# CVMI-Lab/DODA

Measured on AMD Instinct MI355X. Metric: active-voxels/sec fwd+bwd SparseConv U-Net, ScanNet 2cm, higher is better.
Workload: dtype bf16; 1 GPU; cfgs/scannet SparseConv U-Net training step (voxel pooling + fwd + CE + bwd + SGD), 2 cm voxels, 4 scenes/GPU x ~150000 active voxels, random-init weights; global_batch=4, voxels_per_gpu=601279, points_per_gpu=781042, parallelism=dp1, n_classes=20, grad_sync=deferred multi-layer wgrad + bucketed all-reduce, collectives=none (single process), prefetch_gate=off, grad_exchange=no process group

## Files before the change

doda_amd/csrc/spconv_gather.hip:

```cpp
#include <cstdio>
#include "common.hpp"
#include "tilebook.hpp"
#include "spconv_common.hpp"
#include "wgrad_backends.hpp"
#include <stdlib.h>

namespace {

struct F32 {
    typedef float elem;
    typedef f32x4 frag;
    static __device__ __forceinline__ frag zero() { return (frag){0.f, 0.f, 0.f, 0.f}; }
    static __device__ __forceinline__ elem from_float(float f) { return f; }
    static __device__ __forceinline__ float to_float(elem e) { return e; }
    static __device__ __forceinline__ void mma(f32x4 &acc, const frag &w, const frag &x) {
        mma_f32_k16<false>(acc, __builtin_bit_cast(u32x4, w), __builtin_bit_cast(u32x4, x));
    }
    static __device__ __forceinline__ void store4(elem *p, const f32x4 &v) {
        *reinterpret_cast<f32x4 *>(p) = v;
    }
};

struct BF16 {
    typedef unsigned short elem;
    typedef s16x4 frag;
    static __device__ __forceinline__ frag zero() { return (frag){0, 0, 0, 0}; }
    static __device__ __forceinline__ elem from_float(float f) { return f2bf(f); }
    static __device__ __forceinline__ float to_float(elem e) { return __uint_as_float((unsigned)e << 16); }
    static __device__ __forceinline__ void mma(f32x4 &acc, const frag &w, const frag &x) {
        acc = __builtin_amdgcn_mfma_f32_16x16x16bf16_1k(w, x, acc, 0, 0, 0);
    }
    static __device__ __forceinline__ void store4(elem *p, const f32x4 &v) {
        s16x4 o;
#pragma unroll
        for (int q = 0; q < 4; ++q) o[q] = (short)f2bf(v[q]);
        *reinterpret_cast<s16x4 *>(p) = o;
    }
};

template <class T>
__global__ __launch_bounds__(256) void pack_weights(const float *__restrict__ w, int K, int kc,
                                                    int nc, int n_chunk, int NB, int wl,
                                                    typename T::frag *__restrict__ packed) {
    const long long total = (long long)K * n_chunk * NB * 64;
    const long long e = (long long)blockIdx.x * blockDim.x + threadIdx.x;
    if (e >= total) return;
    const int lane = (int)(e & 63);
    long long r = e >> 6;
    const int nb = (int)(r % NB); r /= NB;
    const int cc = (int)(r % n_chunk);
    const int o = (int)(r / n_chunk);
    const int i = lane & 15, g = lane >> 4;
    const int col = nb * 16 + i;
    typename T::frag v;
#pragma unroll
    for (int q = 0; q < 4; ++q) {
        const int c = cc * 16 + 4 * g + q;
        float f = 0.f;
        if (c < kc && col < nc) {
            if (wl == 0) f = w[((long long)o * kc + c) * nc + col];
            else f = w[((long long)(wl == 2 ? K - 1 - o : o) * nc + col) * kc + c];
        }
        v[q] = T::from_float(f);
    }
    packed[e] = v;
}

__device__ __forceinline__ u32x4_t pack_wide_frag(const float *__restrict__ w, int K, int kc, int nc,
                                                  int wl, int o, int cc, int nb, int lane) {
    const int i = lane & 15, g = lane >> 4;
    const int col = nb * 16 + i;
    unsigned short h[8];
#pragma unroll
    for (int q = 0; q < 8; ++q) {
        const int c = cc * 32 + 8 * g + q;
        float f = 0.f;
        if (c < kc && col < nc) {
            if (wl == 0) f = w[((unsigned)o * (unsigned)kc + (unsigned)c) * (unsigned)nc + (unsigned)col];
            else f = w[((unsigned)(wl == 2 ? K - 1 - o : o) * (unsigned)nc + (unsigned)col) * (unsigned)kc + (unsigned)c];
        }
        h[q] = f2bf(f);
    }
    u32x4_t r;
#pragma unroll
    for (int q = 0; q < 4; ++q) r[q] = (unsigned)h[2 * q] | ((unsigned)h[2 * q + 1] << 16);
    return r;
}

__global__ __launch_bounds__(256) void pack_weights_wide(const float *__restrict__ w, int K, int kc,
                                                         int nc, int n_chunk, int NB, int wl,
                                                         u32x4_t *__restrict__ packed, int pair) {
    const long long e = (long long)blockIdx.x * blockDim.x + threadIdx.x;
    if (pair) {
        if (e >= (long long)K * NB * 32) return;
        const long long r = e >> 5;
        packed[e] = pack_wide_frag(w, K, kc, nc, wl, (int)(r / NB), 0, (int)(r % NB), (int)(e & 31));
        return;
    }
    const long long total = (long long)K * n_chunk * NB * 64;
    if (e >= total) return;
    const int lane = (int)(e & 63);
    long long r = e >> 6;
    const int nb = (int)(r % NB); r /= NB;
    const int cc = (int)(r % n_chunk);
    const int o = (int)(r / n_chunk);
    packed[e] = pack_wide_frag(w, K, kc, nc, wl, o, cc, nb, lane);
}

struct PackDesc {
    const float *w;
    void *out;
    int K, kc, nc, layout, elem_bytes, n_chunk, NB, pad;
};

template <class T>
__device__ __forceinline__ void pack_one(const PackDesc &d, long long e) {
    const int lane = (int)(e & 63);
    const unsigned r = (unsigned)(e >> 6), r1 = r / (unsigned)d.NB;
    const int nb = (int)(r - r1 * (unsigned)d.NB);
    const int o = (int)(r1 / (unsigned)d.n_chunk), cc = (int)(r1 - (unsigned)o * (unsigned)d.n_chunk);
    const int i = lane & 15, g = lane >> 4;
    const int col = nb * 16 + i;
    typename T::frag v;
#pragma unroll
    for (int q = 0; q < 4; ++q) {
        const int c = cc * 16 + 4 * g + q;
        float f = 0.f;
        if (c < d.kc && col < d.nc) {
            if ((d.layout & 3) == 0) f = d.w[((long long)o * d.kc + c) * d.nc + col];
            else f = d.w[((long long)((d.layout & 3) == 2 ? d.K - 1 - o : o) * d.nc + col) * d.kc + c];
        }
        v[q] = T::from_float(f);
    }
    reinterpret_cast<typename T::frag *>(d.out)[e] = v;
}

__global__ __launch_bounds__(256) void pack_weights_multi(const PackDesc *__restrict__ descs,
                                                          const int *__restrict__ blk_end, int n_desc) {
    int lo = 0, hi = n_desc - 1;
    while (lo < hi) {
        const int mid = (lo + hi) >> 1;
        if ((int)blockIdx.x < blk_end[mid]) hi = mid; else lo = mid + 1;
    }
    const PackDesc d = descs[lo];
    const int first = lo == 0 ? 0 : blk_end[lo - 1];
    const unsigned e = (unsigned)(blockIdx.x - first) * 256u + threadIdx.x;
    if (d.layout & 0x20) {
        if (e >= (unsigned)d.K * (unsigned)d.NB * 32u) return;
        const unsigned r = e >> 5, o = r / (unsigned)d.NB;
        reinterpret_cast<u32x4_t *>(d.out)[e] =
            pack_wide_frag(d.w, d.K, d.kc, d.nc, d.layout & 3, (int)o, 0, (int)(r - o * (unsigned)d.NB), (int)(e & 31));
        return;
    }
    const unsigned total = (unsigned)d.K * (unsigned)d.n_chunk * (unsigned)d.NB * 64u;
    if (e >= total) return;
    if (d.layout & 0x10) {
        const unsigned r = e >> 6, r1 = r / (unsigned)d.NB, nb = r - r1 * (unsigned)d.NB;
        const unsigned o = r1 / (unsigned)d.n_chunk, cc = r1 - o * (unsigned)d.n_chunk;
        reinterpret_cast<u32x4_t *>(d.out)[e] =
            pack_wide_frag(d.w, d.K, d.kc, d.nc, d.layout & 3, (int)o, (int)cc, (int)nb, (int)(e & 63));
    } else if (d.elem_bytes == 4) pack_one<F32>(d, e);
    else pack_one<BF16>(d, e);
}

constexpr int MAX_K = 27;

template <class T, int NBW, int S>
__global__ __launch_bounds__(256) void conv_gather(const typename T::elem *__restrict__ x, int kc,
                                                   const typename T::frag *__restrict__ wp, int nc,
                                                   int NB, const int32_t *__restrict__ tbl, int ld,
                                                   int K, int n_out,
                                                   typename T::elem *__restrict__ y, int vec_ok,
                                                   const typename T::elem *__restrict__ res) {
    typedef typename T::frag frag;
    typedef typename T::elem elem;
    constexpr int TM = 4 * 16 * S;
    __shared__ int32_t idx_tile[MAX_K * TM];

    const int lane = threadIdx.x & 63, wid = threadIdx.x >> 6;
    const int i = lane & 15, g = lane >> 4;
    const int n_nbg = (NB + NBW - 1) / NBW;
    const int item = xcd_work_item(blockIdx.x, gridDim.x);
    const long long r0 = (long long)(item / n_nbg) * TM;
    const int nb0 = (item % n_nbg) * NBW;

    for (int e = threadIdx.x; e < K * TM; e += 256) {
        const int o = e / TM, r = e - o * TM;
        idx_tile[e] = (r0 + r < n_out) ? tbl[(long long)o * ld + r0 + r] : -1;
    }
    doda_sync();

    const int wrow = wid * 16 * S;
    if (r0 + wrow >= n_out) return;

    unsigned int active = 0;
    for (int o = 0; o < K; ++o) {
        bool any = false;
#pragma unroll
        for (int s = 0; s < S; ++s) any |= idx_tile[o * TM + wrow + s * 16 + i] >= 0;
        if (__ballot(any) != 0ull) active |= 1u << o;
    }
    active = __builtin_amdgcn_readfirstlane(active);

    f32x4 acc[S][NBW];
#pragma unroll
    for (int s = 0; s < S; ++s)
#pragma unroll
        for (int nb = 0; nb < NBW; ++nb) acc[s][nb] = (f32x4){0.f, 0.f, 0.f, 0.f};

    const int n_chunk = (kc + 15) / 16;

    auto load_unit = [&](int o, int cc, frag (&xa)[S], frag (&wb)[NBW]) {
        const int c0 = cc * 16 + 4 * g;
#pragma unroll
        for (int s = 0; s < S; ++s) {
            const int idx = idx_tile[o * TM + wrow + s * 16 + i];
            xa[s] = T::zero();
            if (idx >= 0 && c0 < kc) {
                const elem *row = x + (long long)idx * kc + c0;
                if (vec_ok) {
                    xa[s] = *reinterpret_cast<const frag *>(row);
                } else {
#pragma unroll
                    for (int q = 0; q < 4; ++q)
                        if (c0 + q < kc) xa[s][q] = row[q];
                }
            }
        }
        const frag *wrow_p = wp + (((long long)o * n_chunk + cc) * NB + nb0) * 64 + lane;
#pragma unroll
        for (int nb = 0; nb < NBW; ++nb)
            if (nb0 + nb < NB) wb[nb] = wrow_p[nb * 64];
    };
    auto mma_unit = [&](const frag (&xa)[S], const frag (&wb)[NBW]) {
#pragma unroll
        for (int nb = 0; nb < NBW; ++nb)
#pragma unroll
            for (int s = 0; s < S; ++s) T::mma(acc[s][nb], wb[nb], xa[s]);
    };
    auto advance = [&](int &o, int &cc) -> bool {
        if (++cc < n_chunk) return true;
        cc = 0;
        if (active == 0) return false;
        o = __builtin_ctz(active);
        active &= active - 1;
        return true;
    };

    if (active != 0) {
        frag xa0[S], xa1[S], wb0[NBW], wb1[NBW];
#pragma unroll
        for (int nb = 0; nb < NBW; ++nb) { wb0[nb] = T::zero(); wb1[nb] = T::zero(); }
        int o = __builtin_ctz(active), cc = 0;
        active &= active - 1;
        load_unit(o, cc, xa0, wb0);
        for (;;) {
            const bool m1 = advance(o, cc);
            if (m1) load_unit(o, cc, xa1, wb1);
            mma_unit(xa0, wb0);
            if (!m1) break;
            const bool m0 = advance(o, cc);
            if (m0) load_unit(o, cc, xa0, wb0);
            mma_unit(xa1, wb1);
            if (!m0) break;
        }
    }

#pragma unroll
    for (int s = 0; s < S; ++s) {
        const long long t = r0 + wrow + s * 16 + i;
        if (t < n_out) {
#pragma unroll
            for (int nb = 0; nb < NBW; ++nb) {
                const int col = (nb0 + nb) * 16 + 4 * g;
                if (nb0 + nb < NB) {
                    elem *p = y + t * nc + col;
// ... 761 lines not shown
```

doda_amd/csrc/spconv_wgrad.hip:

```cpp
#include "wgrad_common.hpp"
#include <string.h>
#include <mutex>
#include <vector>

namespace {

constexpr int RT = 64;
constexpr int MAX_OGW = 7;
constexpr int PAD = 8;

struct F32 {
    typedef float elem;
    typedef f32x4 frag;
    typedef f32x4 vec;
    static constexpr int VEC = 4;
    static constexpr int KSTEPS = RT / 4;
    typedef float kfrag;
    template <int STRIDE>
    static __device__ __forceinline__ void frags(const elem *tile, int g, int i, int col0, kfrag (&out)[KSTEPS]) {
#pragma unroll
        for (int ks = 0; ks < KSTEPS; ++ks) out[ks] = tile[(ks * 4 + g) * STRIDE + col0 + i];
    }
    static __device__ __forceinline__ f32x4 mma(kfrag a, kfrag b, f32x4 c) {
        return __builtin_amdgcn_mfma_f32_16x16x4f32(a, b, c, 0, 0, 0);
// ... 94 lines not shown

    const long long r_begin = (long long)chunk * rows_per_chunk;
    long long r_end = r_begin + rows_per_chunk;
    if (r_end > n_rows) r_end = n_rows;

    elem *my_a = a_tile[wid];

    typedef typename T::vec vec;
    constexpr int VEC = T::VEC, NVA = TA * 16 / VEC, NVB = TB * 16 / VEC;
    auto load_vec = [&](const elem *p, const elem *safe, int c, int cmax, bool ok) -> vec {
        const bool live = ok && c < cmax;
        if constexpr (VOK) {
            return *reinterpret_cast<const vec *>(live ? p : safe);
        } else {
            vec v = vec{};
            if (live) {
                elem tmp[VEC];
#pragma unroll
                for (int q = 0; q < VEC; ++q) tmp[q] = (c + q < cmax) ? p[q] : (elem)0;
                v = *reinterpret_cast<const vec *>(tmp);
            }
            return v;
        }
    };
    auto gather_row = [&](int idx, vec (&dst)[NVA]) {
#pragma unroll
        for (int f = 0; f < NVA; ++f) {
            const int c = ca0 + f * VEC;
            dst[f] = load_vec(a + (long long)(idx >= 0 ? idx : 0) * ca + c, a, c, ca, idx >= 0);
        }
    };

    constexpr int NDY = (RT * NVB + 255) / 256;
    vec dy_reg[NDY];
    int idx_n[OGW];
    auto load_dy = [&](long long r0) {
#pragma unroll
        for (int k = 0; k < NDY; ++k) {
            const int e = threadIdx.x + k * 256;
            const int r = e / NVB, f = e - r * NVB;
            const long long row = r0 + r;
            const int c = cb0 + f * VEC;
            dy_reg[k] = load_vec(b + (row < r_end ? row : 0) * cb + c, b, c, cb, e < RT * NVB && row < r_end);
        }
    };
    auto load_idx = [&](long long r0) {
#pragma unroll
        for (int oo = 0; oo < OGW; ++oo) {
            const int o = o_base + wid + 4 * oo;
            const long long row = r0 + lane;
            idx_n[oo] = tbl[(o < K && row < r_end) ? (long long)o * ld + row : 0];
        }
    };

    vec rows_cur[NVA], rows_nxt[NVA];
    if (r_begin < r_end) {
        load_dy(r_begin);
        load_idx(r_begin);
        gather_row((o_base + wid < K && r_begin + lane < r_end) ? idx_n[0] : -1, rows_cur);
    }
    for (long long r0 = r_begin; r0 < r_end; r0 += RT) {
        doda_sync();
#pragma unroll
        for (int k = 0; k < NDY; ++k) {
            const int e = threadIdx.x + k * 256;
            if (e < RT * NVB) {
                const int r = e / NVB, f = e - r * NVB;
                const bool live = r0 + r < r_end && cb0 + f * VEC < cb;
                *reinterpret_cast<vec *>(&b_tile[r * SB + f * VEC]) = (VOK && !live) ? vec{} : dy_reg[k];
            }
        }
        int idx[OGW];
#pragma unroll
        for (int oo = 0; oo < OGW; ++oo)
            idx[oo] = (o_base + wid + 4 * oo < K && r0 + lane < r_end) ? idx_n[oo] : -1;
        const bool more = r0 + RT < r_end;
        if (more) {
            load_dy(r0 + RT);
            load_idx(r0 + RT);
        }
        doda_sync();
        kfrag bf[TB][T::KSTEPS];
#pragma unroll
        for (int y_ = 0; y_ < TB; ++y_) T::template frags<SB>(b_tile, g, i, y_ * 16, bf[y_]);

#pragma unroll
        for (int oo = 0; oo < OGW; ++oo) {
            if (oo + 1 < OGW) gather_row(idx[oo + 1], rows_nxt);
            else if (more) gather_row((o_base + wid < K && r0 + RT + lane < r_end) ? idx_n[0] : -1, rows_nxt);
            if (__ballot(idx[oo] >= 0) != 0ull) {
#pragma unroll
                for (int f = 0; f < NVA; ++f) {
                    const bool live = idx[oo] >= 0 && ca0 + f * VEC < ca;
                    *reinterpret_cast<vec *>(&my_a[lane * SA + f * VEC]) = (VOK && !live) ? vec{} : rows_cur[f];
                }
                __builtin_amdgcn_wave_barrier();
#pragma unroll
                for (int x_ = 0; x_ < TA; ++x_) {
                    kfrag af[T::KSTEPS];
                    T::template frags<SA>(my_a, g, i, x_ * 16, af);
#pragma unroll
                    for (int ks = 0; ks < T::KSTEPS; ++ks)
#pragma unroll
                        for (int y_ = 0; y_ < TB; ++y_)
                            acc[oo][x_][y_] = T::mma(af[ks], bf[y_][ks], acc[oo][x_][y_]);
                }
                __builtin_amdgcn_wave_barrier();
            }
#pragma unroll
            for (int f = 0; f < NVA; ++f) rows_cur[f] = rows_nxt[f];
        }
    }

    float *out = partial + (long long)chunk * K * ca * cb;
#pragma unroll
    for (int oo = 0; oo < OGW; ++oo) {
        const int o = o_base + wid + 4 * oo;
        if (o < K) {
#pragma unroll
            for (int x_ = 0; x_ < TA; ++x_)
#pragma unroll
                for (int y_ = 0; y_ < TB; ++y_)
#pragma unroll
                    for (int r = 0; r < 4; ++r) {
                        const int ci = ca0 + x_ * 16 + 4 * g + r, co = cb0 + y_ * 16 + i;
                        if (ci < ca && co < cb)
                            out[((long long)o * ca + ci) * cb + co] = acc[oo][x_][y_][r];
                    }
        }
    }
}

struct WJob {
    const void *a, *b;
    const int32_t *tbl;
    float *out;
    int ca, cb, ld, K, n_rows, rows_per_chunk, n_tag, n_tbg, n_og, blk_end;
};
using doda_wgrad::RJob;

template <class T, int TA, int TB, int OGW, bool VOK>
__global__ __launch_bounds__(256) void wgrad_multi_kernel(const WJob *__restrict__ jobs, int n_jobs) {
    const int j = find_job<WJob, &WJob::blk_end>(jobs, n_jobs, (int)blockIdx.x);
    const WJob d = jobs[j];
    const int first = j == 0 ? 0 : jobs[j - 1].blk_end;
    wgrad_body<T, TA, TB, OGW, VOK>((const typename T::elem *)d.a, d.ca, (const typename T::elem *)d.b, d.cb,
                                    d.tbl, d.ld, d.K, d.n_rows, d.rows_per_chunk, d.n_tag, d.n_tbg, d.n_og,
                                    d.out, (int)blockIdx.x - first);
}

__global__ __launch_bounds__(256) void wgrad_reduce_multi(const RJob *__restrict__ jobs, int n_jobs) {
    const int j = find_job<RJob, &RJob::blk_end>(jobs, n_jobs, (int)blockIdx.x);
    const RJob d = jobs[j];
    wgrad_fold((int)blockIdx.x - (j == 0 ? 0 : jobs[j - 1].blk_end), d.R, d.n_quad, d.n_quad, d.dw, d.accumulate,
               [&](long long q) { return d.partial + q; });
}

__global__ __launch_bounds__(256) void wgrad_reduce(const float *__restrict__ partial, int R,
                                                    long long n_elem, float *__restrict__ dw,
                                                    int accumulate = 0) {
    __shared__ float part[16][17];
    const int el = threadIdx.x & 15, rl = threadIdx.x >> 4;
    const long long e = (long long)blockIdx.x * 16 + el;
    float s = 0.f;
    if (e < n_elem)
        for (int r = rl; r < R; r += 16) s += partial[(long long)r * n_elem + e];
    part[rl][el] = s;
    doda_sync();
    if (rl == 0 && e < n_elem) {
        float t = 0.f;
#pragma unroll
        for (int r = 0; r < 16; ++r) t += part[r][el];
        dw[e] = accumulate ? dw[e] + t : t;
    }
}


static_assert(WP_RT == RT && WP_MAX_OGW == MAX_OGW, "wgrad_plan.hpp restates these constants");

template <class T, WgradPolicy P, class... Tile>
void launch_multi_variant(WgradTiles<Tile...>, const DensePlan &p, int total_blocks, const WJob *jobs_dev, int n, hipStream_t s) {
    const auto go = [&](auto tile) {
        typedef decltype(tile) Tl;
        if constexpr (dense_compiled(P, Tl::TA, Tl::TB, Tl::OGW))
            if (p.TA == Tl::TA && p.TB == Tl::TB && p.OGW == Tl::OGW)
                with_bool(p.vok, [&](auto vok) {
                    hipLaunchKernelGGL((wgrad_multi_kernel<T, Tl::TA, Tl::TB, Tl::OGW, decltype(vok)::value>), dim3(total_blocks), dim3(256), 0, s, jobs_dev, n);
                });
    };
    (go(Tile{}), ...);
}

struct Staging {
    std::mutex mu;
    void *host = nullptr;
    size_t cap = 0;
    hipEvent_t ev = nullptr;
    int ev_dev = -1;
    bool pending = false;
};
Staging g_staging;

namespace doda_dense {

struct Plan {
    std::vector<int> idx;
    std::vector<DensePlan> jp;
    std::vector<size_t> ws_off;
    std::vector<char> red;
    struct Group { int first, count, blocks, rep; };
    std::vector<Group> groups;
    std::vector<int> order, blk_end;
    int status = DODA_OK;
    size_t partial_bytes = 0, desc_bytes = 0;
    int n_reduce = 0;
};

Plan plan(const doda_wgrad_job *jobs, const std::vector<int> &idx) {
    Plan p;
    p.idx = idx;
    p.jp.resize(idx.size());
    p.ws_off.resize(idx.size());
    p.red.resize(idx.size());
    std::vector<int> keys;
    for (size_t k = 0; k < idx.size(); ++k) {
        DensePlan &jp = p.jp[k];
        const doda_wgrad_job &j = jobs[idx[k]];
        jp.key = -1;
        if (!dense_valid(j)) { p.status = DODA_ERR_INVALID; continue; }
        jp = plan_dense(j, doda_wgrad::switches());
        if (!dense_compiled(jp.policy, jp.TA, jp.TB, jp.OGW) && p.status == DODA_OK) p.status = DODA_ERR_UNSUPPORTED;
        const bool quads = (long long)j.K * j.ca * j.cb % 4 == 0 && (uintptr_t)j.dw % 16 == 0;
        p.red[k] = !dense_needs_partial(jp, j) ? 0 : quads ? 1 : 2;
        p.ws_off[k] = p.partial_bytes;
        p.partial_bytes += dense_partial_bytes(jp, j);
        p.n_reduce += p.red[k] == 1;
        bool seen = false;
        for (int key : keys) seen |= key == jp.key;
        if (!seen) keys.push_back(jp.key);
    }
    for (int key : keys) {
        Plan::Group g{(int)p.order.size(), 0, 0, -1};
        for (size_t k = 0; k < idx.size(); ++k) {
            if (p.jp[k].key != key) continue;
            if (g.rep < 0) g.rep = (int)k;
            g.blocks += p.jp[k].blocks;
            p.order.push_back((int)k);
            p.blk_end.push_back(g.blocks);
            ++g.count;
        }
        p.groups.push_back(g);
    }
    p.desc_bytes = p.order.size() * sizeof(WJob);
    return p;
}

void write_desc(const Plan &p, const doda_wgrad_job *jobs, char *part, void *desc, std::vector<RJob> &reduce, int *reduce_blocks) {
    WJob *wj = (WJob *)desc;
    for (size_t q = 0; q < p.order.size(); ++q) {
        const int k = p.order[q];
        const DensePlan &jp = p.jp[k];
        const doda_wgrad_job &j = jobs[p.idx[k]];
        WJob d;
        d.a = j.a; d.b = j.b; d.tbl = j.tbl;
        d.out = p.red[k] ? (float *)(part + p.ws_off[k]) : j.dw;
        d.ca = j.ca; d.cb = j.cb; d.ld = j.ld; d.K = j.K; d.n_rows = j.n_rows;
        d.rows_per_chunk = jp.rows_per_chunk; d.n_tag = jp.n_tag; d.n_tbg = jp.n_tbg; d.n_og = jp.n_og;
        d.blk_end = p.blk_end[q];
        wj[q] = d;
    }
    for (size_t k = 0; k < p.idx.size(); ++k)
        if (p.red[k] == 1) doda_wgrad::push_reduce(reduce, reduce_blocks, part + p.ws_off[k], jobs[p.idx[k]], p.jp[k].R);
}

int launch(const Plan &p, const void *desc_dev, hipStream_t s) {
    const WJob *wj_dev = (const WJob *)desc_dev;
    for (const Plan::Group &g : p.groups) {
        const DensePlan &q = p.jp[g.rep];
        char name[64];
        dense_name(q, name, sizeof name);
        doda_wgrad::trace(name, g.blocks, 256, g.count);
        if (q.policy == WP_F32S) launch_multi_variant<F32S, WP_F32S>(DenseTiles{}, q, g.blocks, wj_dev + g.first, g.count, s);
        else if (q.policy == WP_F32) launch_multi_variant<F32, WP_F32>(DenseTiles{}, q, g.blocks, wj_dev + g.first, g.count, s);
        else launch_multi_variant<BF16, WP_BF16>(DenseTiles{}, q, g.blocks, wj_dev + g.first, g.count, s);
    }
    return doda_check_launch();
}

int launch_scalar_reduce(const Plan &p, const doda_wgrad_job *jobs, char *part, hipStream_t s) {
    for (size_t k = 0; k < p.idx.size(); ++k) {
        const doda_wgrad_job &j = jobs[p.idx[k]];
        const long long n_elem = (long long)j.K * j.ca * j.cb;
        if (p.red[k] != 2) continue;
        doda_wgrad::trace("wgrad_reduce", div_up(n_elem, 16), 256, 1);
        hipLaunchKernelGGL(wgrad_reduce, dim3(div_up(n_elem, 16)), dim3(256), 0, s, (const float *)(part + p.ws_off[k]), p.jp[k].R,
                           n_elem, j.dw, (j.flags & DODA_WGRAD_ACCUMULATE) ? 1 : 0);
    }
    return doda_check_launch();
}

}

struct CallPlan {
    std::vector<int> cls;
    doda_dense::Plan dense;
    doda_pairs::Plan pairs;
    doda_wdma::Plan tile;
// ... 101 lines not shown
```

doda_amd/csrc/spconv_wwide.hip:

```cpp
#include "wgrad_common.hpp"
#include "tilebook.hpp"
#include <string.h>
#include <algorithm>
#include <vector>

namespace {

constexpr int WW_WAVES = 16;
constexpr int WW_MO = (TB_K + WW_WAVES - 1) / WW_WAVES;
constexpr int WW_LIST_BYTES = TB_UMAX * 4;
constexpr int ww_stage_bytes(int ta, int tb) { return TB_T * 32 * tb + (TB_LMAX + 1) * 32 * ta; }
constexpr int WW_STAGE_MAX = ww_stage_bytes(3, 3);
constexpr int WW_SMEM = WW_LIST_BYTES + TB_LIDX_BYTES + WW_STAGE_MAX;
static_assert(WW_SMEM <= 160 * 1024, "one workgroup per CU");
static_assert(TB_T + 1 <= TB_LMAX + 1, "the dense fallback stages 256 rows into the row slots");

struct WwJob {
    const unsigned short *x, *dy;
    const int32_t *tbl;
    const void *tb;
    float *dw, *part;
    int ca, cb, ld, n_rows, nt, ta, tb_, n_sb, P, rpc, accumulate;
    int wg_end, red_end;
    int pad;
};

__device__ __forceinline__ s16x4 ww_tr(unsigned addr) {
    return __builtin_amdgcn_ds_read_tr16_b64_v4i16((__attribute__((address_space(3))) s16x4 *)(uintptr_t)addr);
}
__device__ __forceinline__ bf16x8 ww_frag(unsigned a_lo, unsigned a_hi) {
    const s16x4 lo = ww_tr(a_lo), hi = ww_tr(a_hi);
    return __builtin_bit_cast(bf16x8, __builtin_shufflevector(lo, hi, 0, 1, 2, 3, 4, 5, 6, 7));
}

template <int TA, int TB>
__device__ void ww_body(const WwJob &d, int local, unsigned char *smem) {
    constexpr int RA = 32 * TA, RB = 32 * TB;
    constexpr int CIS = 16 * TA, COS = 16 * TB, SLICE = TB_K * CIS * COS;
    const int tid = threadIdx.x, wid = __builtin_amdgcn_readfirstlane(tid >> 6);
    const int lane = tid & 63, i = lane & 15, g = lane >> 4, q4 = i >> 2, c4 = i & 3;
    const int slice = local / d.P, p = local - slice * d.P;
    const int sa = slice / d.n_sb, sb = slice - sa * d.n_sb;
    const int ca0 = sa * CIS, cb0 = sb * COS;
    const int r_begin = p * d.rpc, r_end = min(d.n_rows, r_begin + d.rpc);
    const int tile_begin = r_begin / TB_T, tile_end = (r_end - 1) / TB_T + 1;
    static_assert(ww_stage_bytes(TA, TB) <= WW_STAGE_MAX, "staging buffers");
    const int32_t *tb_ulist = (const int32_t *)d.tb;
    const uint32_t *tb_lidx = (const uint32_t *)(tb_ulist + (size_t)d.nt * TB_UMAX);
    const int32_t *tb_ucount = (const int32_t *)(tb_lidx + (size_t)d.nt * (TB_LIDX_BYTES / 4));

    int32_t *list_s = reinterpret_cast<int32_t *>(smem);
    const unsigned *lidx_s = reinterpret_cast<const unsigned *>(smem + WW_LIST_BYTES);
    unsigned char *dy_s = smem + WW_LIST_BYTES + TB_LIDX_BYTES;
    unsigned char *rows_s = dy_s + TB_T * RB;
    const unsigned dy_base = (unsigned)(uintptr_t)dy_s, rows_base = (unsigned)(uintptr_t)rows_s;

    f32x4 acc[WW_MO][TA][TB];
#pragma unroll
    for (int m = 0; m < WW_MO; ++m)
#pragma unroll
        for (int a = 0; a < TA; ++a)
#pragma unroll
            for (int b = 0; b < TB; ++b) acc[m][a][b] = (f32x4){0.f, 0.f, 0.f, 0.f};

    auto multiply = [&](bool dense, int only_o, int ks_begin, int ks_end) {
#pragma unroll 1
        for (int ks = ks_begin; ks < ks_end; ++ks) {
            const int r = 32 * ks + 8 * g + q4;
            bf16x8 bf[TB];
#pragma unroll
            for (int b = 0; b < TB; ++b) {
                const unsigned a0 = dy_base + (unsigned)(r * RB + b * 32 + c4 * 8);
                bf[b] = ww_frag(a0, a0 + 4u * RB);
            }
#pragma unroll
            for (int m = 0; m < WW_MO; ++m) {
                const int o = wid + WW_WAVES * m;
                if (o >= TB_K || (dense && o != only_o)) continue;
                unsigned s0, s1;
                if (dense) {
                    s0 = (unsigned)(r + 1);
                    s1 = (unsigned)(r + 5);
                } else {
                    const unsigned *pl = lidx_s + tb_lplane(o) * TB_T;
                    const unsigned sh = tb_lshift(o);
                    s0 = __builtin_amdgcn_ubfe(pl[tb_lpos(r)], sh, 10u);
                    s1 = __builtin_amdgcn_ubfe(pl[tb_lpos(r + 4)], sh, 10u);
                }
                const unsigned x0 = rows_base + s0 * RA + (unsigned)(c4 * 8), x1 = rows_base + s1 * RA + (unsigned)(c4 * 8);
#pragma unroll
                for (int a = 0; a < TA; ++a) {
                    const bf16x8 af = ww_frag(x0 + 32u * a, x1 + 32u * a);
#pragma unroll
                    for (int b = 0; b < TB; ++b)
                        acc[m][a][b] = __builtin_amdgcn_mfma_f32_16x16x32_bf16(af, bf[b], acc[m][a][b], 0, 0, 0);
                }
            }
        }
    };

    for (int e = tid; e < RA / 16; e += 1024) reinterpret_cast<u32x4 *>(rows_s)[e] = (u32x4){0u, 0u, 0u, 0u};
    for (int tile = tile_begin; tile < tile_end; ++tile) {
        const int t0 = tile * TB_T;
        const int ks_begin = max(0, (r_begin - t0) / 32), ks_end = min(TB_T / 32, (r_end - t0 + 31) / 32);
        const int ucount = tb_ucount[tile];
        const bool listed = ucount <= TB_LMAX;
        if (listed) {
            const int e = (tid & 3) * 256 + ((tid >> 7) & 7) * 32 + ((tid >> 2) & 31);
            list_s[e] = tb_ulist[(size_t)tile * TB_UMAX + tid];
            for (int v = tid; v < TB_LIDX_BYTES / 16; v += 1024)
                reinterpret_cast<u32x4 *>(smem + WW_LIST_BYTES)[v] =
                    reinterpret_cast<const u32x4 *>(tb_lidx + (size_t)tile * (TB_LIDX_BYTES / 4))[v];
        }
        for (int v = tid; v < TB_T * (RB / 16); v += 1024) {
            const int t = v / (RB / 16), f = v - t * (RB / 16);
            u32x4 val = (u32x4){0u, 0u, 0u, 0u};
            if (t0 + t < d.n_rows) val = *reinterpret_cast<const u32x4 *>(d.dy + (size_t)(t0 + t) * d.cb + cb0 + f * 8);
            *reinterpret_cast<u32x4 *>(dy_s + t * RB + f * 16) = val;
        }
        doda_sync();
        if (listed) {
            for (int v = tid; v < ucount * (RA / 16); v += 1024) {
                const int e = v / (RA / 16), f = v - e * (RA / 16);
                const int row = list_s[e];
                *reinterpret_cast<u32x4 *>(rows_s + (e + 1) * RA + f * 16) =
                    *reinterpret_cast<const u32x4 *>(d.x + (size_t)row * d.ca + ca0 + f * 8);
            }
            doda_sync();
            multiply(false, 0, ks_begin, ks_end);
            doda_sync();
        } else {
            for (int o = 0; o < TB_K; ++o) {
                for (int v = tid; v < TB_T * (RA / 16); v += 1024) {
                    const int t = v / (RA / 16), f = v - t * (RA / 16);
                    const int row = t0 + t < d.n_rows ? d.tbl[(size_t)o * d.ld + t0 + t] : -1;
                    u32x4 val = (u32x4){0u, 0u, 0u, 0u};
                    if (row >= 0) val = *reinterpret_cast<const u32x4 *>(d.x + (size_t)row * d.ca + ca0 + f * 8);
                    *reinterpret_cast<u32x4 *>(rows_s + (t + 1) * RA + f * 16) = val;
                }
                doda_sync();
                multiply(true, o, ks_begin, ks_end);
                doda_sync();
            }
        }
    }

    float *dst = d.part + (size_t)local * SLICE;
#pragma unroll
    for (int m = 0; m < WW_MO; ++m) {
        const int o = wid + WW_WAVES * m;
        if (o >= TB_K) continue;
#pragma unroll
        for (int a = 0; a < TA; ++a)
#pragma unroll
            for (int b = 0; b < TB; ++b)
#pragma unroll
                for (int r = 0; r < 4; ++r)
                    dst[((size_t)o * CIS + a * 16 + 4 * g + r) * COS + b * 16 + i] = acc[m][a][b][r];
    }
}

__global__ __launch_bounds__(1024) void wgrad_wide(const WwJob *__restrict__ jobs, int n_jobs) {
    __shared__ __attribute__((aligned(16))) unsigned char smem[WW_SMEM];
    const int j = find_job<WwJob, &WwJob::wg_end>(jobs, n_jobs, (int)blockIdx.x);
    const WwJob d = jobs[j];
    const int local = (int)blockIdx.x - (j == 0 ? 0 : jobs[j - 1].wg_end);
#define WW_CASE(A, B) if (d.ta == A && d.tb_ == B) { ww_body<A, B>(d, local, smem); return; }
    WW_SHAPES(WW_CASE)
#undef WW_CASE
}

__global__ __launch_bounds__(256) void wgrad_wide_reduce(const WwJob *__restrict__ jobs, int n_jobs) {
    const int j = find_job<WwJob, &WwJob::red_end>(jobs, n_jobs, (int)blockIdx.x);
    const WwJob d = jobs[j];
    const int CIS = 16 * d.ta, COS = 16 * d.tb_, SLICE = TB_K * CIS * COS;
    wgrad_fold((int)blockIdx.x - (j == 0 ? 0 : jobs[j - 1].red_end), d.P, (long long)TB_K * d.ca * d.cb / 4, SLICE / 4,
               reinterpret_cast<float4 *>(d.dw), d.accumulate, [&](long long q) {
        const long long e = 4 * q;
        const int co = (int)(e % d.cb), ci = (int)((e / d.cb) % d.ca), o = (int)(e / ((long long)d.ca * d.cb));
        const int slice = (ci / CIS) * d.n_sb + co / COS;
        return reinterpret_cast<const float4 *>(d.part + ((size_t)slice * d.P) * SLICE + ((size_t)o * CIS + ci % CIS) * COS + co % COS);
    });
}

}

namespace doda_wwide {

Plan plan(const doda_wgrad_job *jobs, const std::vector<int> &idx) {
    Plan pl;
    pl.n = (int)idx.size();
    std::vector<int> order;
    for (int k = 0; k < pl.n; ++k) order.push_back(k);
    std::stable_sort(order.begin(), order.end(), [&](int a, int b) { return jobs[idx[a]].n_rows > jobs[idx[b]].n_rows; });
    std::vector<WwJob> desc;
    for (int kk : order) {
        const doda_wgrad_job &j = jobs[idx[kk]];
        WwJob d;
        d.x = (const unsigned short *)j.a; d.dy = (const unsigned short *)j.b; d.tbl = j.tbl; d.tb = j.tilebook;
        d.dw = j.dw;
        d.ca = j.ca; d.cb = j.cb; d.ld = j.ld; d.n_rows = j.n_rows; d.nt = (j.n_rows + TB_T - 1) / TB_T;
        const WideGeo g = wwide_geo(j, doda_wgrad::switches());
        d.ta = g.ta; d.tb_ = g.tb; d.rpc = g.rpc; d.P = g.P;
        d.n_sb = j.cb / (16 * d.tb_);
        d.accumulate = (j.flags & DODA_WGRAD_ACCUMULATE) ? 1 : 0;
        d.part = (float *)(uintptr_t)pl.partial_bytes;
        pl.partial_bytes += g.partial_bytes;
        pl.wgs += g.blocks;
        d.wg_end = pl.wgs;
        pl.red_blocks += doda_wgrad::reduce_blocks((long long)TB_K * j.ca * j.cb / 4, d.P);
        d.red_end = pl.red_blocks;
        d.pad = 0;
        desc.push_back(d);
    }
    pl.desc_bytes = desc.size() * sizeof(WwJob);
    pl.desc.resize(pl.desc_bytes);
    if (pl.desc_bytes) memcpy(pl.desc.data(), desc.data(), pl.desc_bytes);
    return pl;
}

size_t desc_bytes_per_job() { return sizeof(WwJob); }

void write_desc(const Plan &p, char *part, void *desc) {
    if (p.desc_bytes) memcpy(desc, p.desc.data(), p.desc_bytes);
    WwJob *d = (WwJob *)desc;
    for (int k = 0; k < p.n; ++k) d[k].part = (float *)(part + (uintptr_t)d[k].part);
}

int launch(const Plan &p, const void *desc_dev, hipStream_t s) {
    doda_wgrad::trace("wgrad_wide", p.wgs, 1024, p.n);
    hipLaunchKernelGGL(wgrad_wide, dim3(p.wgs), dim3(1024), 0, s, (const WwJob *)desc_dev, p.n);
    doda_wgrad::trace("wgrad_wide_reduce", p.red_blocks, 256, p.n);
    hipLaunchKernelGGL(wgrad_wide_reduce, dim3(p.red_blocks), dim3(256), 0, s, (const WwJob *)desc_dev, p.n);
    return doda_check_launch();
}

}
```

doda_amd/csrc/voxelize.hip:

```cpp
#include "common.hpp"

namespace {

__global__ __launch_bounds__(256) void voxel_pool_fwd(const float *__restrict__ feats,
                                                      float *__restrict__ out,
                                                      const int32_t *__restrict__ rules,
                                                      int n_rows, int row_w, int n_plane,
                                                      int average) {
    const long long total = (long long)n_rows * n_plane;
    for (long long e = (long long)blockIdx.x * blockDim.x + threadIdx.x; e < total;
         e += (long long)gridDim.x * blockDim.x) {
        const int row = (int)(e / n_plane), plane = (int)(e - (long long)row * n_plane);
        const int32_t *r = rules + (long long)row * row_w;
        const int cnt = r[0];
        const float mult = (average && cnt > 0) ? __fdiv_rn(1.0f, (float)cnt) : 1.0f;
        float acc = out[e];
        for (int i = 1; i <= cnt; ++i) {
            const float v = feats[(long long)r[i] * n_plane + plane];
            acc = __fadd_rn(acc, __fmul_rn(mult, v));
        }
        out[e] = acc;
    }
}

__global__ __launch_bounds__(256) void voxel_pool_bwd(const float *__restrict__ d_out,
                                                      float *__restrict__ d_feats,
                                                      const int32_t *__restrict__ rules,
                                                      int n_rows, int row_w, int n_plane,
                                                      int average) {
    const long long total = (long long)n_rows * n_plane;
    for (long long e = (long long)blockIdx.x * blockDim.x + threadIdx.x; e < total;
         e += (long long)gridDim.x * blockDim.x) {
        const int row = (int)(e / n_plane), plane = (int)(e - (long long)row * n_plane);
        const int32_t *r = rules + (long long)row * row_w;
        const int cnt = r[0];
        const float mult = (average && cnt > 0) ? __fdiv_rn(1.0f, (float)cnt) : 1.0f;
        const float g = __fmul_rn(mult, d_out[e]);
        for (int i = 1; i <= cnt; ++i) atomicAdd(&d_feats[(long long)r[i] * n_plane + plane], g);
    }
}

template <typename OUT>
__global__ __launch_bounds__(256) void voxel_pool_rows(const float *__restrict__ fa, int ca, const float *__restrict__ fb, int cb,
                                                       const int32_t *__restrict__ rules, int n_rows, int row_w, int average,
                                                       OUT *__restrict__ out, int c_out) {
    const long long total = (long long)n_rows * c_out;
    for (long long e = (long long)blockIdx.x * blockDim.x + threadIdx.x; e < total; e += (long long)gridDim.x * blockDim.x) {
        const int row = (int)(e / c_out), plane = (int)(e - (long long)row * c_out);
        float acc = 0.0f;
        if (plane < ca + cb) {
            const int32_t *r = rules + (long long)row * row_w;
            const int cnt = r[0];
            const float mult = (average && cnt > 0) ? __fdiv_rn(1.0f, (float)cnt) : 1.0f;
            const bool first = plane < ca;
            const float *src = first ? fa + plane : fb + (plane - ca);
            const int ld = first ? ca : cb;
            for (int i = 1; i <= cnt; ++i) acc = __fadd_rn(acc, __fmul_rn(mult, src[(long long)r[i] * ld]));
        }
        if constexpr (sizeof(OUT) == 2) out[e] = __builtin_bit_cast(unsigned short, (__bf16)acc);
        else out[e] = acc;
    }
}

template <typename OUT>
__global__ __launch_bounds__(256) void voxel_pool_rows_lane(const float *__restrict__ fa, int ca, const float *__restrict__ fb, int cb,
                                                            const int32_t *__restrict__ rules, int n_rows, int row_w, int average,
                                                            OUT *__restrict__ out, int c_out) {
    typedef unsigned int u32x4_ __attribute__((ext_vector_type(4)));
    constexpr int EPP = 16 / (int)sizeof(OUT);
    const int pieces = c_out / EPP;
    for (int row = blockIdx.x * blockDim.x + threadIdx.x; row < n_rows; row += gridDim.x * blockDim.x) {
        const int32_t *r = rules + (long long)row * row_w;
        const int cnt = r[0];
        const float mult = (average && cnt > 0) ? __fdiv_rn(1.0f, (float)cnt) : 1.0f;
        float acc[8];
#pragma unroll
        for (int c = 0; c < 8; ++c) acc[c] = 0.0f;
        for (int i = 1; i <= cnt; ++i) {
            const long long p = r[i];
#pragma unroll
            for (int c = 0; c < 8; ++c) {
                if (c < ca) acc[c] = __fadd_rn(acc[c], __fmul_rn(mult, fa[p * ca + c]));
                else if (c < ca + cb) acc[c] = __fadd_rn(acc[c], __fmul_rn(mult, fb[p * cb + (c - ca)]));
            }
        }
        u32x4_ *o = reinterpret_cast<u32x4_ *>(out + (long long)row * c_out);
        if constexpr (sizeof(OUT) == 2) {
            u32x4_ v;
#pragma unroll
            for (int k = 0; k < 4; ++k)
                v[k] = (unsigned)__builtin_bit_cast(unsigned short, (__bf16)acc[2 * k]) |
                       ((unsigned)__builtin_bit_cast(unsigned short, (__bf16)acc[2 * k + 1]) << 16);
            o[0] = v;
            for (int k = 1; k < pieces; ++k) o[k] = (u32x4_){0u, 0u, 0u, 0u};
        } else {
            o[0] = (u32x4_){__float_as_uint(acc[0]), __float_as_uint(acc[1]), __float_as_uint(acc[2]), __float_as_uint(acc[3])};
            if (pieces > 1) o[1] = (u32x4_){__float_as_uint(acc[4]), __float_as_uint(acc[5]), __float_as_uint(acc[6]), __float_as_uint(acc[7])};
            for (int k = 2; k < pieces; ++k) o[k] = (u32x4_){0u, 0u, 0u, 0u};
        }
    }
}

int launch_pool(bool fwd, const float *src, float *dst, const int32_t *rules, int average,
                int n_active, int max_active, int n_plane, doda_stream_t stream) {
    if (n_active < 0 || max_active < 0 || n_plane < 0) return DODA_ERR_INVALID;
    if (n_active == 0 || n_plane == 0) return DODA_OK;
    if (!src || !dst || !rules) return DODA_ERR_INVALID;
    const long long total = (long long)n_active * n_plane;
    const int grid = (int)((total + 255) / 256 < 256 * 16 ? (total + 255) / 256 : 256 * 16);
    if (fwd)
        hipLaunchKernelGGL(voxel_pool_fwd, dim3(grid), dim3(256), 0, as_stream(stream), src, dst,
                           rules, n_active, max_active + 1, n_plane, average);
    else
        hipLaunchKernelGGL(voxel_pool_bwd, dim3(grid), dim3(256), 0, as_stream(stream), src, dst,
                           rules, n_active, max_active + 1, n_plane, average);
    return doda_check_launch();
}
}

extern "C" int doda_voxelize_fp(const float *feats, float *out, const int32_t *rules, int32_t mode,
                                int32_t n_active, int32_t max_active, int32_t n_plane,
                                doda_stream_t stream) {
    return launch_pool(true, feats, out, rules, mode == 4, n_active, max_active, n_plane, stream);
}

extern "C" int doda_voxelize_bp(const float *d_out, float *d_feats, const int32_t *rules,
                                int32_t mode, int32_t n_active, int32_t max_active,
                                int32_t n_plane, doda_stream_t stream) {
    return launch_pool(false, d_out, d_feats, rules, mode == 4, n_active, max_active, n_plane,
                       stream);
}

extern "C" int doda_voxelize_fp_rows(const float *feats_a, int32_t c_a, const float *feats_b, int32_t c_b, const int32_t *rules,
                                     int32_t mode, int32_t n_active, int32_t max_active, void *out, int32_t c_out,
                                     int32_t out_elem_bytes, doda_stream_t stream) {
    if (n_active < 0 || max_active < 0 || c_a < 1 || c_b < 0 || c_out < c_a + c_b || (out_elem_bytes != 2 && out_elem_bytes != 4) ||
        (c_b > 0 && !feats_b))
        return DODA_ERR_INVALID;
    if (n_active == 0) return DODA_OK;
    if (!feats_a || !rules || !out) return DODA_ERR_INVALID;
    if (c_a + c_b <= 8 && (c_out * out_elem_bytes) % 16 == 0 && (c_out * out_elem_bytes >= 32 || c_a + c_b <= 16 / out_elem_bytes) &&
        ((uintptr_t)out & 15) == 0) {
        const int grid = (n_active + 255) / 256 < 256 * 16 ? (n_active + 255) / 256 : 256 * 16;
        if (out_elem_bytes == 2)
            hipLaunchKernelGGL(voxel_pool_rows_lane<unsigned short>, dim3(grid), dim3(256), 0, as_stream(stream), feats_a, (int)c_a,
                               feats_b, (int)c_b, rules, (int)n_active, (int)max_active + 1, (int)(mode == 4), (unsigned short *)out,
                               (int)c_out);
        else
            hipLaunchKernelGGL(voxel_pool_rows_lane<float>, dim3(grid), dim3(256), 0, as_stream(stream), feats_a, (int)c_a, feats_b,
                               (int)c_b, rules, (int)n_active, (int)max_active + 1, (int)(mode == 4), (float *)out, (int)c_out);
        return doda_check_launch();
    }
    const long long total = (long long)n_active * c_out;
    const int grid = (int)((total + 255) / 256 < 256 * 32 ? (total + 255) / 256 : 256 * 32);
    if (out_elem_bytes == 2)
        hipLaunchKernelGGL(voxel_pool_rows<unsigned short>, dim3(grid), dim3(256), 0, as_stream(stream), feats_a, (int)c_a, feats_b,
                           (int)c_b, rules, (int)n_active, (int)max_active + 1, (int)(mode == 4), (unsigned short *)out, (int)c_out);
    else
        hipLaunchKernelGGL(voxel_pool_rows<float>, dim3(grid), dim3(256), 0, as_stream(stream), feats_a, (int)c_a, feats_b, (int)c_b,
                           rules, (int)n_active, (int)max_active + 1, (int)(mode == 4), (float *)out, (int)c_out);
    return doda_check_launch();
}

extern "C" int doda_point_recover_fp(const float *feats, float *out, const int32_t *rules,
                                     int32_t n_active, int32_t max_active, int32_t n_plane,
                                     doda_stream_t stream) {
    return launch_pool(false, feats, out, rules, 0, n_active, max_active, n_plane, stream);
}

extern "C" int doda_point_recover_bp(const float *d_out, float *d_feats, const int32_t *rules,
                                     int32_t n_active, int32_t max_active, int32_t n_plane,
                                     doda_stream_t stream) {
    return launch_pool(true, d_out, d_feats, rules, 0, n_active, max_active, n_plane, stream);
}
```

doda_amd/csrc/wgrad_common.hpp:

```cpp
#pragma once
#include "wgrad_backends.hpp"

typedef float f32x4 __attribute__((ext_vector_type(4)));
typedef short s16x4 __attribute__((ext_vector_type(4)));
typedef __bf16 bf16x8 __attribute__((ext_vector_type(8)));
typedef unsigned int u32x4 __attribute__((ext_vector_type(4)));

namespace {

template <class J, int J::*END>
__device__ __forceinline__ int find_job(const J *jobs, int n_jobs, int blk) {
    int lo = 0, hi = n_jobs - 1;
    while (lo < hi) {
        const int mid = (lo + hi) >> 1;
        if (blk < jobs[mid].*END) hi = mid; else lo = mid + 1;
    }
    return lo;
}

__device__ __forceinline__ bf16x8 pack_hi16(const f32x4 &d0, const f32x4 &d1) {
    u32x4 r;
    r[0] = __builtin_amdgcn_perm(__float_as_uint(d0[1]), __float_as_uint(d0[0]), 0x07060302u);
    r[1] = __builtin_amdgcn_perm(__float_as_uint(d0[3]), __float_as_uint(d0[2]), 0x07060302u);
    r[2] = __builtin_amdgcn_perm(__float_as_uint(d1[1]), __float_as_uint(d1[0]), 0x07060302u);
    r[3] = __builtin_amdgcn_perm(__float_as_uint(d1[3]), __float_as_uint(d1[2]), 0x07060302u);
    return __builtin_bit_cast(bf16x8, r);
}

template <class Src>
__device__ __forceinline__ void wgrad_fold(int blk, int R, long long n_quad, long long stride, float4 *dw, int accumulate,
                                           Src src) {
    __shared__ float4 part[256];
    const int RL = doda_wgrad::reduce_lanes(R), EL = 256 / RL;
    const int el = (int)threadIdx.x % EL, rl = (int)threadIdx.x / EL;
    const long long q = (long long)blk * EL + el;
    float4 s = make_float4(0.f, 0.f, 0.f, 0.f);
    if (q < n_quad) {
        const float4 *p = src(q);
        for (int r = rl; r < R; r += RL) {
            const float4 v = p[(long long)r * stride];
            s.x += v.x; s.y += v.y; s.z += v.z; s.w += v.w;
        }
    }
    part[rl * EL + el] = s;
    doda_sync();
    if (rl == 0 && q < n_quad) {
        float4 t = part[el];
        for (int r = 1; r < RL; ++r) {
            const float4 v = part[r * EL + el];
            t.x += v.x; t.y += v.y; t.z += v.z; t.w += v.w;
        }
        if (accumulate) {
            const float4 old = dw[q];
            t.x += old.x; t.y += old.y; t.z += old.z; t.w += old.w;
        }
        dw[q] = t;
    }
}

}
```

Before: 138.2 million voxels/s.

## Vectorize weight packing, batch wgrad reductions, specialize voxel pooling loads

Weight pack kernels gain a vectorized f32x4 path for transposed layouts when kc is divisible and the pointer is aligned. The wgrad fold reduction batches independent loads per lane, hoists the accumulate read and skips shared-memory reduction when there is a single lane. The wide-reduce index math swaps 64-bit div/mod for float-reciprocal small division. Voxel pooling gets specialized channel counts that load packed rows and batch several points per iteration. Together these target load latency and integer-division overhead in the small auxiliary kernels, at the cost of extra code paths and a precision-sensitive division trick.

```diff
diff --git a/doda_amd/csrc/spconv_gather.hip b/doda_amd/csrc/spconv_gather.hip
--- a/doda_amd/csrc/spconv_gather.hip
+++ b/doda_amd/csrc/spconv_gather.hip
@@ -37,6 +37,18 @@
         *reinterpret_cast<s16x4 *>(p) = o;
     }
 };
+
+template <int N>
+__device__ __forceinline__ bool pack_run_vec(const float *w, int kc) { return (kc % N) == 0 && ((uintptr_t)w & 15) == 0; }
+template <int N>
+__device__ __forceinline__ void pack_run_load(const float *__restrict__ run, bool inside, float (&f)[N]) {
+#pragma unroll
+    for (int q = 0; q < N; q += 4) {
+        f32x4 v = (f32x4){0.f, 0.f, 0.f, 0.f};
+        if (inside) v = *reinterpret_cast<const f32x4 *>(run + q);
+        f[q] = v[0]; f[q + 1] = v[1]; f[q + 2] = v[2]; f[q + 3] = v[3];
+    }
+}
 
 template <class T>
 __global__ __launch_bounds__(256) void pack_weights(const float *__restrict__ w, int K, int kc,
@@ -53,6 +65,15 @@
     const int i = lane & 15, g = lane >> 4;
     const int col = nb * 16 + i;
     typename T::frag v;
+    if (wl != 0 && pack_run_vec<4>(w, kc)) {
+        const int c = cc * 16 + 4 * g;
+        float f[4];
+        pack_run_load<4>(w + ((long long)(wl == 2 ? K - 1 - o : o) * nc + col) * kc + c, c < kc && col < nc, f);
+#pragma unroll
+        for (int q = 0; q < 4; ++q) v[q] = T::from_float(f[q]);
+        packed[e] = v;
+        return;
+    }
 #pragma unroll
     for (int q = 0; q < 4; ++q) {
         const int c = cc * 16 + 4 * g + q;
@@ -71,15 +92,24 @@
     const int i = lane & 15, g = lane >> 4;
     const int col = nb * 16 + i;
     unsigned short h[8];
-#pragma unroll
-    for (int q = 0; q < 8; ++q) {
-        const int c = cc * 32 + 8 * g + q;
-        float f = 0.f;
-        if (c < kc && col < nc) {
-            if (wl == 0) f = w[((unsigned)o * (unsigned)kc + (unsigned)c) * (unsigned)nc + (unsigned)col];
-            else f = w[((unsigned)(wl == 2 ? K - 1 - o : o) * (unsigned)nc + (unsigned)col) * (unsigned)kc + (unsigned)c];
-        }
-        h[q] = f2bf(f);
+    if (wl != 0 && pack_run_vec<8>(w, kc)) {
+        const int c = cc * 32 + 8 * g;
+        float f[8];
+        pack_run_load<8>(w + ((unsigned)(wl == 2 ? K - 1 - o : o) * (unsigned)nc + (unsigned)col) * (unsigned)kc + (unsigned)c,
+                         c < kc && col < nc, f);
+#pragma unroll
+        for (int q = 0; q < 8; ++q) h[q] = f2bf(f[q]);
+    } else {
+#pragma unroll
+        for (int q = 0; q < 8; ++q) {
+            const int c = cc * 32 + 8 * g + q;
+            float f = 0.f;
+            if (c < kc && col < nc) {
+                if (wl == 0) f = w[((unsigned)o * (unsigned)kc + (unsigned)c) * (unsigned)nc + (unsigned)col];
+                else f = w[((unsigned)(wl == 2 ? K - 1 - o : o) * (unsigned)nc + (unsigned)col) * (unsigned)kc + (unsigned)c];
+            }
+            h[q] = f2bf(f);
+        }
     }
     u32x4_t r;
 #pragma unroll
@@ -122,6 +152,15 @@
     const int i = lane & 15, g = lane >> 4;
     const int col = nb * 16 + i;
     typename T::frag v;
+    if ((d.layout & 3) != 0 && pack_run_vec<4>(d.w, d.kc)) {
+        const int c = cc * 16 + 4 * g;
+        float f[4];
+        pack_run_load<4>(d.w + ((long long)((d.layout & 3) == 2 ? d.K - 1 - o : o) * d.nc + col) * d.kc + c, c < d.kc && col < d.nc, f);
+#pragma unroll
+        for (int q = 0; q < 4; ++q) v[q] = T::from_float(f[q]);
+        reinterpret_cast<typename T::frag *>(d.out)[e] = v;
+        return;
+    }
 #pragma unroll
     for (int q = 0; q < 4; ++q) {
         const int c = cc * 16 + 4 * g + q;
diff --git a/doda_amd/csrc/spconv_wgrad.hip b/doda_amd/csrc/spconv_wgrad.hip
--- a/doda_amd/csrc/spconv_wgrad.hip
+++ b/doda_amd/csrc/spconv_wgrad.hip
@@ -270,7 +270,7 @@
 __global__ __launch_bounds__(256) void wgrad_reduce_multi(const RJob *__restrict__ jobs, int n_jobs) {
     const int j = find_job<RJob, &RJob::blk_end>(jobs, n_jobs, (int)blockIdx.x);
     const RJob d = jobs[j];
-    wgrad_fold((int)blockIdx.x - (j == 0 ? 0 : jobs[j - 1].blk_end), d.R, d.n_quad, d.n_quad, d.dw, d.accumulate,
+    wgrad_fold<8>((int)blockIdx.x - (j == 0 ? 0 : jobs[j - 1].blk_end), d.R, d.n_quad, d.n_quad, d.dw, d.accumulate,
                [&](long long q) { return d.partial + q; });
 }
 
diff --git a/doda_amd/csrc/spconv_wwide.hip b/doda_amd/csrc/spconv_wwide.hip
--- a/doda_amd/csrc/spconv_wwide.hip
+++ b/doda_amd/csrc/spconv_wwide.hip
@@ -14,6 +14,7 @@
 constexpr int WW_SMEM = WW_LIST_BYTES + TB_LIDX_BYTES + WW_STAGE_MAX;
 static_assert(WW_SMEM <= 160 * 1024, "one workgroup per CU");
 static_assert(TB_T + 1 <= TB_LMAX + 1, "the dense fallback stages 256 rows into the row slots");
+static_assert((long long)TB_K * 224 * 224 < (1 << 22), "wgrad_wide_reduce divides element indices with div_small (wwide_eligible: <= 224 channels)");
 
 struct WwJob {
     const unsigned short *x, *dy;
@@ -173,13 +174,15 @@
 __global__ __launch_bounds__(256) void wgrad_wide_reduce(const WwJob *__restrict__ jobs, int n_jobs) {
     const int j = find_job<WwJob, &WwJob::red_end>(jobs, n_jobs, (int)blockIdx.x);
     const WwJob d = jobs[j];
-    const int CIS = 16 * d.ta, COS = 16 * d.tb_, SLICE = TB_K * CIS * COS;
-    wgrad_fold((int)blockIdx.x - (j == 0 ? 0 : jobs[j - 1].red_end), d.P, (long long)TB_K * d.ca * d.cb / 4, SLICE / 4,
+    const unsigned CIS = 16 * d.ta, COS = 16 * d.tb_, SLICE = TB_K * CIS * COS, cab = (unsigned)d.ca * (unsigned)d.cb;
+    const float r_ab = __builtin_amdgcn_rcpf((float)cab), r_b = __builtin_amdgcn_rcpf((float)d.cb);
+    const float r_cis = __builtin_amdgcn_rcpf((float)CIS), r_cos = __builtin_amdgcn_rcpf((float)COS);
+    wgrad_fold<4>((int)blockIdx.x - (j == 0 ? 0 : jobs[j - 1].red_end), d.P, (long long)TB_K * d.ca * d.cb / 4, SLICE / 4,
                reinterpret_cast<float4 *>(d.dw), d.accumulate, [&](long long q) {
-        const long long e = 4 * q;
-        const int co = (int)(e % d.cb), ci = (int)((e / d.cb) % d.ca), o = (int)(e / ((long long)d.ca * d.cb));
-        const int slice = (ci / CIS) * d.n_sb + co / COS;
-        return reinterpret_cast<const float4 *>(d.part + ((size_t)slice * d.P) * SLICE + ((size_t)o * CIS + ci % CIS) * COS + co % COS);
+        unsigned rem, co, cil, col;
+        const unsigned o = div_small(4u * (unsigned)q, cab, r_ab, &rem), ci = div_small(rem, (unsigned)d.cb, r_b, &co);
+        const unsigned sa = div_small(ci, CIS, r_cis, &cil), sb = div_small(co, COS, r_cos, &col);
+        return reinterpret_cast<const float4 *>(d.part + ((size_t)(sa * (unsigned)d.n_sb + sb) * d.P) * SLICE + (o * CIS + cil) * COS + col);
     });
 }
 
diff --git a/doda_amd/csrc/voxelize.hip b/doda_amd/csrc/voxelize.hip
--- a/doda_amd/csrc/voxelize.hip
+++ b/doda_amd/csrc/voxelize.hip
@@ -62,28 +62,70 @@
     }
 }
 
-template <typename OUT>
-__global__ __launch_bounds__(256) void voxel_pool_rows_lane(const float *__restrict__ fa, int ca, const float *__restrict__ fb, int cb,
-                                                            const int32_t *__restrict__ rules, int n_rows, int row_w, int average,
-                                                            OUT *__restrict__ out, int c_out) {
+constexpr int VP_BATCH = 4;
+template <int W> struct __attribute__((packed, aligned(4))) VpRow { float v[W]; };
+
+template <int CA, int CB>
+__device__ __forceinline__ void vp_load_point(const float *__restrict__ fa, int ca, const float *__restrict__ fb, int cb, long long p,
+                                              float (&v)[8]) {
+    if constexpr (CA > 0) {
+        const VpRow<CA> a = *reinterpret_cast<const VpRow<CA> *>(fa + p * CA);
+#pragma unroll
+        for (int c = 0; c < CA; ++c) v[c] = a.v[c];
+        if constexpr (CB > 0) {
+            const VpRow<CB> b = *reinterpret_cast<const VpRow<CB> *>(fb + p * CB);
+#pragma unroll
+            for (int c = 0; c < CB; ++c) v[CA + c] = b.v[c];
+        }
+    } else {
+#pragma unroll
+        for (int c = 0; c < 8; ++c) {
+            if (c < ca) v[c] = fa[p * ca + c];
+            else if (c < ca + cb) v[c] = fb[p * cb + (c - ca)];
+        }
+    }
+}
+
+template <int CA, int CB, int B>
+__device__ __forceinline__ void vp_pool_row(const float *__restrict__ fa, int ca, const float *__restrict__ fb, int cb,
+                                            const int32_t *__restrict__ r, int row_w, int average, float (&acc)[8]) {
+    const int nc = CA > 0 ? CA + CB : ca + cb;
+    const int cnt = r[0];
+    int p[B];
+#pragma unroll
+    for (int k = 0; k < B; ++k) p[k] = 1 + k < row_w ? r[1 + k] : 0;
+    const float mult = (average && cnt > 0) ? __fdiv_rn(1.0f, (float)cnt) : 1.0f;
+#pragma unroll
+    for (int c = 0; c < 8; ++c) acc[c] = 0.0f;
+    for (int i0 = 1; i0 <= cnt; i0 += B) {
+        if (i0 > 1) {
+#pragma unroll
+            for (int k = 0; k < B; ++k) p[k] = r[min(i0 + k, cnt)];
+        }
+        float v[B][8];
+#pragma unroll
+        for (int k = 0; k < B; ++k) vp_load_point<CA, CB>(fa, ca, fb, cb, (long long)(i0 + k <= cnt ? p[k] : p[0]), v[k]);
+#pragma unroll
+        for (int k = 0; k < B; ++k)
+            if (i0 + k <= cnt) {
+#pragma unroll
+                for (int c = 0; c < 8; ++c)
+                    if (c < nc) acc[c] = __fadd_rn(acc[c], __fmul_rn(mult, v[k][c]));
+            }
+    }
+}
+
+template <typename OUT, int CA, int CB, int B>
+__device__ __forceinline__ void vp_rows_lane(const float *__restrict__ fa, int ca, const float *__restrict__ fb, int cb,
+                                             const int32_t *__restrict__ rules, int n_rows, int row_w, int average,
+                                             OUT *__restrict__ out, int c_out) {
     typedef unsigned int u32x4_ __attribute__((ext_vector_type(4)));
     constexpr int EPP = 16 / (int)sizeof(OUT);
     const int pieces = c_out / EPP;
     for (int row = blockIdx.x * blockDim.x + threadIdx.x; row < n_rows; row += gridDim.x * blockDim.x) {
         const int32_t *r = rules + (long long)row * row_w;
-        const int cnt = r[0];
-        const float mult = (average && cnt > 0) ? __fdiv_rn(1.0f, (float)cnt) : 1.0f;
         float acc[8];
-#pragma unroll
-        for (int c = 0; c < 8; ++c) acc[c] = 0.0f;
-        for (int i = 1; i <= cnt; ++i) {
-            const long long p = r[i];
-#pragma unroll
-            for (int c = 0; c < 8; ++c) {
-                if (c < ca) acc[c] = __fadd_rn(acc[c], __fmul_rn(mult, fa[p * ca + c]));
-                else if (c < ca + cb) acc[c] = __fadd_rn(acc[c], __fmul_rn(mult, fb[p * cb + (c - ca)]));
-            }
-        }
+        vp_pool_row<CA, CB, B>(fa, ca, fb, cb, r, row_w, average, acc);
         u32x4_ *o = reinterpret_cast<u32x4_ *>(out + (long long)row * c_out);
         if constexpr (sizeof(OUT) == 2) {
             u32x4_ v;
@@ -99,6 +141,15 @@
             for (int k = 2; k < pieces; ++k) o[k] = (u32x4_){0u, 0u, 0u, 0u};
         }
     }
+}
+
+template <typename OUT>
+__global__ __launch_bounds__(256) void voxel_pool_rows_lane(const float *__restrict__ fa, int ca, const float *__restrict__ fb, int cb,
+                                                            const int32_t *__restrict__ rules, int n_rows, int row_w, int average,
+                                                            OUT *__restrict__ out, int c_out) {
+    if (ca == 3 && cb == 3) vp_rows_lane<OUT, 3, 3, VP_BATCH>(fa, ca, fb, cb, rules, n_rows, row_w, average, out, c_out);
+    else if (ca == 3 && cb == 0) vp_rows_lane<OUT, 3, 0, VP_BATCH>(fa, ca, fb, cb, rules, n_rows, row_w, average, out, c_out);
+    else vp_rows_lane<OUT, 0, 0, 1>(fa, ca, fb, cb, rules, n_rows, row_w, average, out, c_out);
 }
 
 int launch_pool(bool fwd, const float *src, float *dst, const int32_t *rules, int average,
diff --git a/doda_amd/csrc/wgrad_common.hpp b/doda_amd/csrc/wgrad_common.hpp
--- a/doda_amd/csrc/wgrad_common.hpp
+++ b/doda_amd/csrc/wgrad_common.hpp
@@ -27,33 +27,54 @@
     return __builtin_bit_cast(bf16x8, r);
 }
 
-template <class Src>
+__device__ __forceinline__ unsigned div_small(unsigned n, unsigned d, float rd, unsigned *rem) {
+    const unsigned q = (unsigned)((float)n * rd);
+    const int r = (int)(n - q * d), lo = r < 0 ? 1 : 0, hi = r >= (int)d ? 1 : 0;
+    *rem = (unsigned)(r + (lo - hi) * (int)d);
+    return q - lo + hi;
+}
+
+__device__ __forceinline__ void wgrad_add4(float4 &s, const float4 &v) { s.x += v.x; s.y += v.y; s.z += v.z; s.w += v.w; }
+
+template <int BATCH, class Src>
 __device__ __forceinline__ void wgrad_fold(int blk, int R, long long n_quad, long long stride, float4 *dw, int accumulate,
                                            Src src) {
     __shared__ float4 part[256];
-    const int RL = doda_wgrad::reduce_lanes(R), EL = 256 / RL;
-    const int el = (int)threadIdx.x % EL, rl = (int)threadIdx.x / EL;
-    const long long q = (long long)blk * EL + el;
-    float4 s = make_float4(0.f, 0.f, 0.f, 0.f);
-    if (q < n_quad) {
-        const float4 *p = src(q);
-        for (int r = rl; r < R; r += RL) {
-            const float4 v = p[(long long)r * stride];
-            s.x += v.x; s.y += v.y; s.z += v.z; s.w += v.w;
+    const int RL = doda_wgrad::reduce_lanes(R), lr = __builtin_ctz(RL), lg = 8 - lr, EL = 1 << lg;
+    const int el = (int)threadIdx.x & (EL - 1), rl = (int)threadIdx.x >> lg;
+    const long long q = ((long long)blk << lg) + el;
+    const bool live = q < n_quad, owner = live && rl == 0;
+    float4 s = make_float4(0.f, 0.f, 0.f, 0.f), old = s;
+    if (owner && accumulate) old = dw[q];
+    if (live && rl < R) {
+        const float4 *p = src(q) + (long long)rl * stride;
+        if (R <= 16) {
+            wgrad_add4(s, *p);
+        } else {
+            const long long step = (long long)RL * stride;
+#pragma unroll 1
+            for (int n = (R - rl + RL - 1) >> lr; n > 0; n -= BATCH) {
+                float4 v[BATCH];
+#pragma unroll
+                for (int k = 0; k < BATCH; ++k)
+                    if (k < n) { v[k] = *p; p += step; }
+#pragma unroll
+                for (int k = 0; k < BATCH; ++k)
+                    if (k < n) wgrad_add4(s, v[k]);
+            }
         }
     }
-    part[rl * EL + el] = s;
-    doda_sync();
-    if (rl == 0 && q < n_quad) {
-        float4 t = part[el];
-        for (int r = 1; r < RL; ++r) {
-            const float4 v = part[r * EL + el];
-            t.x += v.x; t.y += v.y; t.z += v.z; t.w += v.w;
+    float4 t = s;
+    if (RL > 1) {
+        part[threadIdx.x] = s;
+        doda_sync();
+        if (owner) {
+            t = part[el];
+            for (int r = 1; r < RL; ++r) wgrad_add4(t, part[(r << lg) + el]);
         }
-        if (accumulate) {
-            const float4 old = dw[q];
-            t.x += old.x; t.y += old.y; t.z += old.z; t.w += old.w;
-        }
+    }
+    if (owner) {
+        if (accumulate) wgrad_add4(t, old);
         dw[q] = t;
     }
 }
```

New measurement: 137.5 million voxels/s. About the same (-0.5%).
